# qurAI-amsterdam/SuperResolution_aniso_MRI

Hardware: AMD Instinct MI355X
Metric: training slices/sec (ae_combined, 160x160, latent=128) (higher is better)
Workload: dtype f32; 1 GPU; ACDC synthetic 12x(3x1x160x160) triplets, ae_combined latent=128 depth=32 scales=2, MSE synthesis loss (BASELINE configs[1]); global_batch_triplets=12, parallelism=dp1, init=reference Initializer, seed 892372, random weights, launch=captured HIP graph replay

## Files before the change

### superresolution_aniso_mri_amd/_hip.py

```python
import ctypes
import os
from ctypes import c_char_p, c_double, c_float, c_int, c_int64, c_size_t, c_void_p

import torch

_HERE = os.path.dirname(os.path.abspath(__file__))
LIB_PATH = os.path.join(_HERE, "libaesr_hip.so")
if os.environ.get("AESR_LIB"):
    import sys as _sys
    LIB_PATH = os.path.abspath(os.environ["AESR_LIB"])
    _sys.stderr.write("[aesr] AESR_LIB: loading the VARIANT library %s (not the shipped libaesr_hip.so)\n" % LIB_PATH)

P = c_void_p
IP = ctypes.POINTER(c_int)
FP = ctypes.POINTER(c_float)
DP = ctypes.POINTER(c_double)

class TripletDesc(ctypes.Structure):
    _fields_ = [("vol_off", ctypes.c_longlong), ("H", c_int), ("W", c_int), ("z_from", c_int), ("z_to", c_int), ("z_between", c_int),
                ("oy", c_int), ("ox", c_int), ("k", c_int), ("gain", c_float), ("cutoff", c_float)]


class WgradReduceJob(ctypes.Structure):
    _fields_ = [("workspace", c_void_p), ("dw", c_void_p), ("db", c_void_p), ("N", c_int), ("H", c_int), ("W", c_int), ("Cin", c_int),
# ... 124 lines not shown
    "aesr_comm_unique_id": (c_int, [c_char_p]),
    "aesr_comm_init": (c_int, [c_char_p, c_int, c_int, ctypes.POINTER(c_void_p)]),
    "aesr_comm_destroy": (c_int, [P]),
    "aesr_comm_abort": (c_int, [P]),
    "aesr_comm_allreduce": (c_int, [P, P, c_size_t, c_int, c_int, P]),
    "aesr_comm_allreduce_many": (c_int, [P, ctypes.POINTER(c_void_p), ctypes.POINTER(c_size_t), c_int, c_int, c_int, P]),
    "aesr_comm_broadcast": (c_int, [P, P, c_size_t, c_int, c_int, P]),
}
SIGNATURES_PREPROC = {
    "aesr_inplane_out_size": (c_int, [c_int, c_double]),
    "aesr_inplane_workspace_bytes": (c_size_t, [c_int, c_int]),
    "aesr_inplane_resample": (c_int, [P, P, P] + [c_int] * 5 + [DP, c_int, DP, c_int, IP, DP, IP, DP, c_int, P]),
}
SIGNATURES_DATAPREP = {
    "aesr_thick_slices_out_slices": (c_int, [c_int, c_int]),
    "aesr_thick_slices_store_bytes": (c_int, [c_int, P, P]),
    "aesr_thick_slices": (c_int, [P, P, c_int, c_int, c_int, c_int, DP, c_int, P]),
    "aesr_triplet_assemble_raw": (c_int, [P, ctypes.POINTER(TripletDesc), c_int, c_int, P, P, P]),
}
SIGNATURES_TRAIN = {
    "aesr_conv2d_cout1_bwd_workspace_floats": (c_size_t, [c_int]),
    "aesr_conv2d_cout1_bwd": (c_int, [P] * 8 + [c_int] * 5 + [c_float, c_int, c_float, P]),
}
SIGNATURES_BASELINES = {
    "aesr_z_expand_out_slices": (c_int, [c_int, c_int, c_int]),
    "aesr_z_expand_store_bytes": (c_int, [c_int, P, P]),
    "aesr_bspline_coef_bytes": (c_size_t, [c_int] * 4),
    "aesr_bspline_prefilter_z": (c_int, [P, P] + [c_int] * 4 + [P]),
    "aesr_z_expand": (c_int, [P, P, P] + [c_int] * 7 + [IP, DP, c_int, c_int, P]),
}
SIGNATURES_RESLICE = {
    "aesr_reslice_affine": (c_int, [P, P] + [c_int] * 7 + [DP, c_int, P]),
    "aesr_reslice_grid": (c_int, [P, P, P] + [c_int] * 7 + [c_int, P]),
}
SIGNATURES_SEG = {
    "aesr_softmax_dice_workspace_floats": (c_size_t, [c_int] * 4),
    "aesr_softmax_dice_fwd": (c_int, [P, P, c_size_t] + [P] * 5 + [c_int] * 4 + [P]),
    "aesr_softmax_dice_bwd": (c_int, [P, P, c_size_t, P, P, P] + [c_int] * 4 + [P]),
}
LLP = ctypes.POINTER(ctypes.c_longlong)
SIGNATURES_SURFACE = {
    "aesr_surface_workspace_bytes": (c_size_t, [c_int] * 5),
    "aesr_surface_borders": (c_int, [P, P, P, P] + [c_int] * 4 + [IP, c_int, c_int, c_int, P]),
    "aesr_surface_distances": (c_int, [P, P, LLP, P, c_size_t, P] + [c_int] * 6 + [DP, P]),
}
SURFACE_MAX_CLASSES, SURFACE_COUNTS, SURFACE_MAX_W = 8, 7, 4096
# ... 3 lines not shown
ZX_MAX_FACTOR, ZX_MAX_TAPS = 16, 10
P2P_HANDLE_BYTES, P2P_SLOTS = 64, 32
COMM_ID_BYTES = 128
COMM_F32, COMM_F64, COMM_SUM, COMM_MAX = 0, 1, 0, 1

ACT_NONE, ACT_LRELU, ACT_RELU, ACT_SIGMOID = 0, 1, 2, 3
BN_NONE, BN_POOL, BN_UP = 0, 1, 2
RS_POOL, RS_NEAREST, RS_BILINEAR = 1, 2, 3
BN_NWG = 512
REDUCE_MAX_JOBS = 16
MSE_NPART = 512
MSE3_WS = 3 * 256 + 1
LPIPS_NCH = 64


def _load():
    if not os.path.exists(LIB_PATH):
        raise RuntimeError(
            "libaesr_hip.so not found at %s -- build it with `python __graft_entry__.py` (or `make -C "
            "superresolution_aniso_mri_amd/csrc`). The HIP extension is mandatory: there is no CPU/eager fallback." % LIB_PATH)
    lib = ctypes.CDLL(LIB_PATH)
    for name, (res, args) in (list(SIGNATURES.items()) + list(SIGNATURES_PREPROC.items()) + list(SIGNATURES_DATAPREP.items())
                                   + list(SIGNATURES_TRAIN.items()) + list(SIGNATURES_BASELINES.items()) + list(SIGNATURES_RESLICE.items())
                                   + list(SIGNATURES_SEG.items()) + list(SIGNATURES_SURFACE.items())):
        fn = getattr(lib, name, None)
        if fn is None:
            raise RuntimeError("libaesr_hip.so does not export %s (stale build?)" % name)
        fn.restype, fn.argtypes = res, args
    return lib


lib = _load()


def last_error():
    return lib.aesr_last_error_string().decode("utf-8", "replace")


def check(rc, what):
    if rc != 0:
        raise RuntimeError("%s failed (code %d): %s" % (what, rc, last_error()))


def check_device_watchdogs(where):
    nb = int(lib.aesr_bn_fused1_timeouts())
    if nb:
        raise RuntimeError("%s: the one-launch BatchNorm kernel's grid barrier gave up %d time(s) in this process -- its workgroups were not all "
# ... 45 lines not shown
```

### superresolution_aniso_mri_amd/csrc/aesr_api.hip

```cpp
#include <stdarg.h>
#include <stdio.h>
#include <stdlib.h>
#include <string.h>

#include "../../include/aesr_hip.h"
#include "../../include/aesr_hip_dataprep.h"
#include "../../include/aesr_hip_train.h"
#include "aesr_kernels.h"
#include "conv_plan.h"

static thread_local char g_err[512] = "";
void aesr_set_error(const char* fmt, ...) {
    va_list ap;
    va_start(ap, fmt);
    vsnprintf(g_err, sizeof(g_err), fmt, ap);
    va_end(ap);
}

static bool fill_groups(BnGroups* gr, int G, const int* nstart_host) {
    if (G < 1 || G > 4 || !nstart_host) return false;
    gr->G = G;
    for (int i = 0; i <= G; ++i) gr->nstart[i] = nstart_host[i];
    for (int i = G + 1; i < 5; ++i) gr->nstart[i] = nstart_host[G];
    return true;
}

enum { GEOM_OK = 0, GEOM_FILTER, GEOM_DIMS, GEOM_SMALL };
static int conv_geom(int N, int H, int W, int Cin, int Cout, int KS, int pad, int* Ho, int* Wo) {
// ... 752 lines not shown
    AESR_CHECK_ARG(gout && y && mean && invstd && scale && sums && counts_host && coef && dgamma && dbeta && dpre &&
                       bn_bwd_args(&a, gout, y, mean, invstd, scale, coef, nullptr, dpre, N, H, W, C, mode, act, slope, G, nstart_host),
                   "aesr_bn_bwd_apply: bad arguments");
    if (aesr_bn_fused_ok(C, G))
        return aesr_launch_bn_bwd_finalize_apply(sums, counts_host, coef, dgamma, dbeta, G, a, (hipStream_t)stream);
    if (int e = aesr_launch_bn_bwd_finalize(sums, counts_host, coef, dgamma, dbeta, C, G, (hipStream_t)stream)) return e;
    return aesr_launch_bn_bwd_apply(a, (hipStream_t)stream);
}

int aesr_bn_bwd(const float* gout, const float* y, const float* mean, const float* invstd, const float* scale, float* partial,
                const double* counts_host, float* coef, float* dgamma, float* dbeta, float* dpre, int N, int H, int W, int C,
                int mode, int act, float slope, int G, const int* nstart_host, void* stream) {
    BnBwdArgs a;
    AESR_CHECK_ARG(gout && y && mean && invstd && scale && partial && counts_host && coef && dgamma && dbeta && dpre &&
                       bn_bwd_args(&a, gout, y, mean, invstd, scale, coef, partial, dpre, N, H, W, C, mode, act, slope, G, nstart_host),
                   "aesr_bn_bwd: bad arguments");
    AESR_CHECK_ARG((double)N * H * W < 2147483648.0, "aesr_bn_bwd: more than 2^31 pixels");
    if (int e = aesr_launch_bn_bwd_reduce(a, AESR_BN_NWG, (hipStream_t)stream)) return e;
    if (int e = aesr_launch_bn_bwd_reduce_finalize(partial, AESR_BN_NWG, counts_host, coef, dgamma, dbeta, C, G, (hipStream_t)stream))
        return e;
    return aesr_launch_bn_bwd_apply(a, (hipStream_t)stream);
}

int aesr_maxpool2_fwd(const float* x, float* out, int N, int H, int W, int C, void* stream) {
    AESR_CHECK_ARG(x && out && N > 0 && H >= 2 && W >= 2 && C % 4 == 0, "aesr_maxpool2_fwd: bad arguments (C %% 4 == 0, H,W >= 2)");
    return aesr_launch_maxpool2_fwd(x, out, N, H, W, C, (hipStream_t)stream);
}

int aesr_maxpool2_bwd(const float* gout, const float* x, const float* gadd, float* dx, int N, int H, int W, int C, int relu_mask,
                      void* stream) {
    AESR_CHECK_ARG(gout && x && dx && N > 0 && H >= 2 && W >= 2 && C % 4 == 0, "aesr_maxpool2_bwd: bad arguments");
    return aesr_launch_maxpool2_bwd(gout, x, gadd, dx, N, H, W, C, relu_mask, (hipStream_t)stream);
}

int aesr_scale_expand_fwd(const float* x, float* out4, size_t n, const float* ca_host, const float* cb_host, void* stream) {
    AESR_CHECK_ARG(x && out4 && ca_host && cb_host && n > 0 && n < ((size_t)1 << 29), "aesr_scale_expand_fwd: bad arguments");
    return aesr_launch_scale_expand(x, out4, (int)n, ca_host, cb_host, 0, (hipStream_t)stream);
}

int aesr_scale_expand_bwd(const float* d4, float* dx, size_t n, const float* ca_host, void* stream) {
    AESR_CHECK_ARG(d4 && dx && ca_host && n > 0 && n < ((size_t)1 << 29), "aesr_scale_expand_bwd: bad arguments");
    return aesr_launch_scale_expand(d4, dx, (int)n, ca_host, nullptr, 1, (hipStream_t)stream);
}

int aesr_lpips_tap_fwd(const float* f, const float* lin_w, float* partial, int B, int HW, int C, void* stream) {
    AESR_CHECK_ARG(f && lin_w && partial && B > 0 && HW > 0, "aesr_lpips_tap_fwd: bad arguments");
// ... 212 lines not shown
```

### superresolution_aniso_mri_amd/csrc/aesr_kernels.h

```cpp
#pragma once
#include "aesr_common.h"

struct IgemmArgs {
    const float* in; const float* wpk; const float* bias; const float* ysave; float* out;
    int N, H, W, Cin, CinP, Cout, CoutP, Ho, Wo, pad;
    int TI, TH, TW, tiles_y, tiles_x, nitems, dbg;
    int unused_;
    int ksplit;
    float* dbgbuf;
    int act, mask_act;
    float slope;
};
int aesr_launch_conv_igemm(const IgemmArgs& a, int KS, int NB, int MBW, hipStream_t st);
int aesr_launch_conv_ksplit_fixup(const float* partial, const float* bias, const float* ysave, float* out, size_t nelem, int Cout,
                                  int ksplit, int act, int mask_act, float slope, hipStream_t st);
int aesr_launch_pack_weights(const float* w, float* p, int Cout, int Cin, int KS, int KinP, int NoutP, int TN, int transpose, hipStream_t st);

struct WinoArgs {
    const float* in; const float* upk; const float* bias; const float* ysave; float* out;
    int N, H, W, Cin, CinP, Cout, CoutP;
    int TI, THt, TWt;
    int regs_y, regs_x, nitems;
    unsigned m_ncot, m_regs_x, m_regs_y;
    int act, mask_act;
// ... 163 lines not shown
bool aesr_bn_fused1_ok(int N, int H, int W, int C, int pool, int G, int backward);
unsigned aesr_bn_fused_timeouts_impl();
int aesr_launch_bn_stats(const float* y, float* partial, int HW, int C, const BnGroups& gr, int nwg, hipStream_t st);
int aesr_launch_bn_reduce(const float* partial, double* sums, int nwg, int C, int G, hipStream_t st);
int aesr_launch_bn_finalize(const double* sums, const double* counts, const float* gamma, const float* beta, float* rm, float* rv,
                            long long* nbt, float* mean, float* invstd, float* scale, float* shift, int C, int G, float momentum,
                            float eps, int train, int update_running, hipStream_t st);
int aesr_launch_bn_reduce_finalize(const float* partial, int nwg, const double* counts, const float* gamma, const float* beta,
                                   float* running_mean, float* running_var, long long* nbt, float* mean, float* invstd,
                                   float* scale, float* shift, int C, int G, float momentum, float eps, int update_running,
                                   hipStream_t st);
int aesr_launch_bn_bwd_reduce_finalize(const float* partial, int nwg, const double* counts, float* coef, float* dgamma,
                                       float* dbeta, int C, int G, hipStream_t st);
int aesr_launch_bn_apply(const BnApplyArgs& a, hipStream_t st);
int aesr_launch_bn_bwd_reduce(const BnBwdArgs& a, int nwg, hipStream_t st);
int aesr_launch_bn_bwd_finalize(const double* sums, const double* counts, float* coef, float* dgamma, float* dbeta, int C, int G, hipStream_t st);
int aesr_launch_bn_bwd_apply(const BnBwdArgs& a, hipStream_t st);
bool aesr_bn_fused_ok(int C, int G);
int aesr_launch_bn_finalize_apply(const double* sums, const double* counts, const float* gamma, const float* beta, float* running_mean,
                                  float* running_var, long long* nbt, float* mean, float* invstd, float* scale, float* shift, float momentum,
                                  float eps, int update_running, int G, const BnApplyArgs& a, hipStream_t st);
int aesr_launch_bn_bwd_finalize_apply(const double* sums, const double* counts, float* coef, float* dgamma, float* dbeta, int G,
                                      const BnBwdArgs& a, hipStream_t st);

int aesr_launch_lerp_fwd(const float* z, const float* af, const float* at, float* zmix, int B, size_t per, hipStream_t st);
int aesr_launch_lerp_bwd(const float* dmix, const float* af, const float* at, float* dz, int B, size_t per, hipStream_t st);
int aesr_launch_lerp_cat_fwd(const float* z, const float* af, const float* at, float* zcat, int B, size_t per, hipStream_t st);
int aesr_launch_interleave_clamp(const float* orig, const float* synth, float* out, int Z, int n, size_t per, float lo, float hi, hipStream_t st);
int aesr_launch_lerp_multi(const float* z, float* out, int Z, size_t per, const float* alphas, int n, float nslope, hipStream_t st);
int aesr_launch_lerp_cat_bwd(const float* g, const float* af, const float* at, float* dz, int B, size_t per, hipStream_t st);
int aesr_launch_mse_fwd(const float* a, const float* b, double* partial, int np, float* out, size_t n, hipStream_t st);
int aesr_launch_mse3_fwd(const float* const* a, const float* const* b, const size_t* n, const float* lam, double* ws, float* out, hipStream_t st);
int aesr_launch_mse3_bwd(const float* a1, const float* b1, size_t n1, const float* a2, const float* b2, size_t n2, const float* lam,
                         const float* g, float* d1, float* d2, hipStream_t st);
int aesr_launch_mse_bwd(const float* a, const float* b, const float* g, float* da, size_t n, hipStream_t st);
int aesr_launch_act_bwd(const float* dout, const float* y, float* dpre, size_t n, int act, float slope, hipStream_t st);
int aesr_launch_adam(float* p, float* g, float* m, float* v, float* state, size_t n, float lr, double beta1, double beta2,
                     float eps, float wd, int zero_g, hipStream_t st);


int aesr_launch_maxpool2_fwd(const float* x, float* out, int N, int H, int W, int C, hipStream_t st);
int aesr_launch_maxpool2_bwd(const float* gout, const float* x, const float* gadd, float* dx, int N, int H, int W, int C, int relu, hipStream_t st);
int aesr_launch_lpips_tap_fwd(const float* f, const float* lin, float* partial, int B, int HW, int C, hipStream_t st);
int aesr_launch_lpips_tap_bwd(const float* f, const float* lin, const float* gd, float* gf0, int B, int HW, int C, hipStream_t st);
int aesr_launch_lpips_finalize(const float* const* partials, const int* hw, int ntaps, float* d, int B, hipStream_t st);
int aesr_launch_scale_expand(const float* x, float* out4, int n, const float* ca, const float* cb, int backward, hipStream_t st);
// ... 24 lines not shown
```

### superresolution_aniso_mri_amd/csrc/bn.hip

```cpp
#include "bn_math.h"

enum { BN_MODE_NONE = 0, BN_MODE_POOL = 1, BN_MODE_UP = 2 };

__global__ __launch_bounds__(256) void bn_stats_kernel(const float* __restrict__ y, float* __restrict__ partial, int HW,
                                                       int C, BnGroups gr) {
    extern __shared__ __attribute__((aligned(16))) float red[];
    const int C4 = C >> 2, PL = 256 / C4;
    const int c4 = threadIdx.x % C4, pl = threadIdx.x / C4;
    const int g = blockIdx.y;
    const size_t p0 = (size_t)gr.nstart[g] * HW, p1 = (size_t)gr.nstart[g + 1] * HW;
    f32x4 s = {0.f, 0.f, 0.f, 0.f}, q = {0.f, 0.f, 0.f, 0.f};
    if (pl < PL) {
        for (size_t p = p0 + (size_t)blockIdx.x * PL + pl; p < p1; p += (size_t)gridDim.x * PL) {
            const f32x4 v = *(const f32x4*)(y + p * C + c4 * 4);
            s += v;
            q += v * v;
        }
        *(f32x4*)(red + (pl * 2 + 0) * C + c4 * 4) = s;
        *(f32x4*)(red + (pl * 2 + 1) * C + c4 * 4) = q;
    }
    __syncthreads();
    for (int o = threadIdx.x; o < 2 * C; o += 256) {
        float t = 0.f;
        for (int k = 0; k < PL; ++k) t += red[k * 2 * C + o];
// ... 273 lines not shown
        const f32x4 mu = *(const f32x4*)(a.mean + g * a.C + c4 * 4);
        const f32x4 iv = *(const f32x4*)(a.invstd + g * a.C + c4 * 4);
        const f32x4 sc = *(const f32x4*)(a.scale + g * a.C + c4 * 4);
        const f32x4 k1 = *(const f32x4*)(k_tab + (g * 2 + 0) * a.C + c4 * 4);
        const f32x4 k2 = *(const f32x4*)(k_tab + (g * 2 + 1) * a.C + c4 * 4);
        const f32x4 yv = *(const f32x4*)(a.y + idx * 4);
        const f32x4 gg = bn_gather_g_t<MODE>(a, n, yy, x, c4);
        *(f32x4*)(a.dpre + idx * 4) = bn_bwd_elem(yv, gg, mu, iv, sc, k1, k2, a.act, a.slope);
    }
}

template <int MODE>
__global__ __launch_bounds__(256) void bn_bwd_apply_kernel(BnBwdArgs a) { bn_bwd_apply_loop<MODE>(a, a.coef); }

template <int MODE>
__global__ __launch_bounds__(256) void bn_bwd_finalize_apply_kernel(const double* __restrict__ sums, BnCounts counts, float* __restrict__ coef,
                                                                    float* __restrict__ dgamma, float* __restrict__ dbeta, int G, BnBwdArgs a) {
    __shared__ __attribute__((aligned(16))) float s_k[2 * BN_FUSE_MAX];
    bn_bwd_tables<256>(sums, counts.c, G, a.C, blockIdx.x == 0, s_k, coef, dgamma, dbeta);
    __syncthreads();
    bn_bwd_apply_loop<MODE>(a, s_k);
}

static int bn_check_c(int C, const char* who) {
    if (C % 4 != 0 || 256 % (C / 4) != 0 || C > 1024) {
        aesr_set_error("%s: unsupported channel count %d (need C/4 | 256)", who, C);
        return AESR_ERR_ARG;
    }
    return AESR_OK;
}

static dim3 bn_stream_grid(size_t pixels, int C) {
    const size_t total = pixels * (C / 4);
    int grid = (int)((total + 255) / 256);
    if (grid > 4096) grid = 4096;
    return dim3(grid);
}

#define BN_LAUNCH_MODE(kernel, mode, grid, shm, st, ...)                                                       \
    do {                                                                                                       \
        if ((mode) == BN_MODE_POOL) hipLaunchKernelGGL(kernel<BN_MODE_POOL>, grid, dim3(256), shm, st, __VA_ARGS__); \
        else if ((mode) == BN_MODE_UP) hipLaunchKernelGGL(kernel<BN_MODE_UP>, grid, dim3(256), shm, st, __VA_ARGS__);  \
        else hipLaunchKernelGGL(kernel<0>, grid, dim3(256), shm, st, __VA_ARGS__);                             \
    } while (0)

int aesr_launch_bn_stats(const float* y, float* partial, int HW, int C, const BnGroups& gr, int nwg, hipStream_t st) {
// ... 92 lines not shown
}

bool aesr_bn_fused_ok(int C, int G) { return G * C <= BN_FUSE_MAX && G >= 1 && G <= 4; }

int aesr_launch_bn_finalize_apply(const double* sums, const double* counts, const float* gamma, const float* beta, float* running_mean,
                                  float* running_var, long long* nbt, float* mean, float* invstd, float* scale, float* shift, float momentum,
                                  float eps, int update_running, int G, const BnApplyArgs& a, hipStream_t st) {
    if (int e = bn_check_c(a.C, "bn_finalize_apply")) return e;
    const BnFinArgs f = bn_fin_args(counts, gamma, beta, running_mean, running_var, nbt, mean, invstd, scale, shift, a.C, G, momentum, eps, 1,
                                    update_running);
    hipLaunchKernelGGL(bn_finalize_apply_kernel, bn_stream_grid((size_t)a.N * a.Ho * a.Wo, a.C), dim3(256), 0, st, sums, f, a);
    AESR_LAUNCH_CHECK("bn_finalize_apply");
    return AESR_OK;
}

int aesr_launch_bn_bwd_finalize_apply(const double* sums, const double* counts, float* coef, float* dgamma, float* dbeta, int G,
                                      const BnBwdArgs& a, hipStream_t st) {
    if (int e = bn_check_c(a.C, "bn_bwd_finalize_apply")) return e;
    BN_LAUNCH_MODE(bn_bwd_finalize_apply_kernel, a.mode, bn_stream_grid((size_t)a.N * a.H * a.W, a.C), 0, st, sums, bn_counts(counts, G), coef,
                   dgamma, dbeta, G, a);
    AESR_LAUNCH_CHECK("bn_bwd_finalize_apply");
    return AESR_OK;
}
```

### superresolution_aniso_mri_amd/engine.py

```python
import os
from ctypes import c_float

import torch
import torch.nn as nn

from . import _hip
from ._hip import lib, ptr, stream, check

LRELU_SLOPE = 0.01


class KernelProfiler:

    def __init__(self):
        self.records = []

    def begin(self, kind, flops, nbytes=0.0):
        e0 = torch.cuda.Event(enable_timing=True)
        e1 = torch.cuda.Event(enable_timing=True)
        e0.record(torch.cuda.current_stream())
        self.records.append((kind, flops, nbytes, e0, e1))

    def end(self):
        self.records[-1][4].record(torch.cuda.current_stream())

    def summary(self):
        torch.cuda.synchronize()
        out = {}
        for kind, flops, nbytes, e0, e1 in self.records:
            d = out.setdefault(kind, {"launches": 0, "flops": 0.0, "bytes": 0.0, "ms": 0.0})
            d["launches"] += 1
            d["flops"] += flops
            d["bytes"] += nbytes
            d["ms"] += e0.elapsed_time(e1)
        return out


PROFILER = None
TRACE = None
FUSE_STEM = os.environ.get("AESR_FUSE_STEM", "1") != "0"
FUSE_COUT1_BWD = os.environ.get("AESR_FUSE_COUT1_BWD", "1") != "0"
USE_WINO = os.environ.get("AESR_WINO", "1") != "0"
FOLD_UPSAMPLE = os.environ.get("AESR_FOLD_UPSAMPLE", "1") != "0"
FUSE_EVAL_BN = os.environ.get("AESR_FUSE_EVAL_BN", "1") != "0"


def bn_fused_enabled():
    return os.environ.get("AESR_BN_FUSED", "1") != "0"


def bn_fused_pays(N, H, W, C):
    if N > int(os.environ.get("AESR_BN_FUSED_MAX_IMAGES", "9")):
        return False
    return float(N) * H * W * C * 4.0 <= float(os.environ.get("AESR_BN_FUSED_MAX_MB", "1000")) * 1e6


def wino_ok(cin, cout, ks, pad, transpose):
    return bool(USE_WINO and lib.aesr_conv2d_wino_supported(int(cin), int(cout), int(ks), int(pad), int(transpose)))


def wino_kind(n, h, w, cin, cout, transpose):
    k = lib.aesr_conv2d_wino_kernel(int(n), int(h), int(w), int(cin), int(cout), 3, 1, int(transpose))
    return {2: "conv_wino_res_f32", 3: "conv_wino_ring_f32"}.get(k, "conv_wino_f32")

# ... 350 lines not shown
                    check(lib.aesr_conv2d_smallcin_fwd(ptr(cur), ptr(s.mod.weight), ptr(bias), None, ptr(out), N, H, W,
                                                       s.cin, s.cout, s.ks, s.pad, act_k, _hip.ACT_NONE, s.slope, 0, 0,
                                                       None, None, stream()), "aesr_conv2d_smallcin_fwd")
                else:
                    raise NotImplementedError("conv with Cin=%d (neither <=4 nor a multiple of 4)" % s.cin)
                if save:
                    saved.append((cur, out, full_hw) if s.s2d else (cur, out))
                if TRACE is not None and not skip:
                    TRACE.append((self.seq, s.mod, act_k, out))
                cur, H, W, C = out, Ho, Wo, s.cout
            elif s.kind == "resample":
                if C % 4 != 0:
                    raise NotImplementedError("stand-alone pooling / upsampling of %d channels (needs a multiple of 4)" % C)
                Ho, Wo = s.out_hw(H, W)
                out = _empty((N, Ho, Wo, C), x)
                check(lib.aesr_resample2_fwd(ptr(cur), ptr(out), N, H, W, C, s.mode, stream()), "aesr_resample2_fwd")
                if save:
                    saved.append((cur,))
                cur, H, W = out, Ho, Wo
            else:
                bn = s.mod
                Ho, Wo = s.out_hw(H, W)
                out = _empty((N, Ho, Wo, C), x)
                _pb("bn_fwd", 0.0, 4.0 * (cur.numel() + out.numel()))
                st = self._bn_forward_stats(bn, cur, N, H, W, C, nstart, train, out, s.run_mode)
                if not st.pop("applied", False):
                    check(lib.aesr_bn_apply(ptr(cur), ptr(st["scale"]), ptr(st["shift"]), ptr(out), N, H, W, C, s.run_mode, G,
                                            _hip.int_array(nstart), stream()), "aesr_bn_apply")
                _pe()
                if save:
                    saved.append((cur, st))
                cur, H, W = out, Ho, Wo
        return cur, saved, steps

    def max_elems_per_image(self, H, W, C, first=0, last=None):
        return self.trace_shapes(H, W, C, first, last)[0]

    def trace_shapes(self, H, W, C, first=0, last=None):
        best = H * W * C
        for s in self.steps[first:last]:
            if s.kind == "conv":
                if s.s2d:
                    H, W = H // 2, W // 2
                elif s.in_up2:
                    H, W = 2 * H, 2 * W
                    H, W = s.out_hw(H, W)
                else:
                    H, W = s.out_hw(H, W)
# ... 8 lines not shown

    def _bn_barrier(self, dev):
        t = self.__dict__.get("_bn_bar")
        if t is None or t.device != torch.device(dev):
            if torch.cuda.is_current_stream_capturing():
                raise RuntimeError("one-launch BatchNorm: run the pass eagerly once before capturing it into a HIP graph")
            t = self._bn_bar = torch.zeros((int(lib.aesr_bn_fused1_barrier_words()),), device=dev, dtype=torch.int32)
        return t

    sync_p2p = None

    def _p2p_fits(self, N, H, W, C, run_mode, G, backward):
        p = self.sync_p2p
        if p is None or not bn_fused_enabled():
            return False
        nmax = max(N, int(round(N * p.nscale)))
        if float(nmax) * H * W * C * 4.0 > float(os.environ.get("AESR_P2P_MAX_MB", "12")) * 1e6:
            return False
        return bool(lib.aesr_bn_fused1_supported(nmax, H, W, C, run_mode, G, backward))

    sync_bn = None
    count_scale = 1.0

    def _bn_forward_stats(self, bn, y, N, H, W, C, nstart, train, out=None, run_mode=0):
        G = len(nstart) - 1
        dev = y.device
        st = {k: torch.empty((G, C), device=dev, dtype=torch.float32) for k in ("mean", "invstd", "scale", "shift")}
        use_batch = train or bn.running_mean is None
        momentum = 0.1 if bn.momentum is None else float(bn.momentum)
        update = bool(train and bn.track_running_stats and bn.running_mean is not None)
        if update:
            self._bn_updates = getattr(self, "_bn_updates", 0) + 1
        if not use_batch:
            ver = lambda t: (-1, 0) if t is None else (t._version, t.data_ptr())
            key = (self.weights_epoch, getattr(self, "_bn_updates", 0), ver(bn.weight), ver(bn.bias), ver(bn.running_mean), ver(bn.running_var),
                   G, str(dev))
            cache = self.__dict__.setdefault("_eval_bn", {})
            hit = cache.get(id(bn))
            if hit is not None and hit[0] == key and not torch.cuda.is_current_stream_capturing():
                return dict(hit[1])
        sums = None
        counts = [float((nstart[g + 1] - nstart[g]) * H * W) * self.count_scale for g in range(G)] if use_batch else None
        st["counts"] = counts
        if use_batch:
            partial = torch.empty((G * _hip.BN_NWG * 2 * C,), device=dev, dtype=torch.float32)
            local = (self.sync_bn is None and out is not None and bn_fused_enabled() and bn_fused_pays(N, H, W, C)
                     and lib.aesr_bn_fused1_supported(N, H, W, C, run_mode, G, 0))
            if local or (self.sync_bn is not None and out is not None and self._p2p_fits(N, H, W, C, run_mode, G, 0)):
                ws = torch.empty((lib.aesr_bn_fused1_workspace_floats(C, G),), device=dev, dtype=torch.float32)
                args = (ptr(y), ptr(out), ptr(ws), ptr(self._bn_barrier(dev)), _hip.double_array(counts), ptr(bn.weight), ptr(bn.bias),
                        ptr(bn.running_mean), ptr(bn.running_var), ptr(bn.num_batches_tracked), ptr(st["mean"]), ptr(st["invstd"]),
                        ptr(st["scale"]), ptr(st["shift"]), N, H, W, C, run_mode, G, _hip.int_array(nstart), momentum, float(bn.eps), int(update))
                if local:
                    check(lib.aesr_bn_fused1_fwd(*args, stream()), "aesr_bn_fused1_fwd")
                else:
                    p = self.sync_p2p
                    check(lib.aesr_bn_fused1_fwd_p2p(*args, p.peers, p.world, p.rank, p.next_slot(), ptr(p.gen), stream()), "aesr_bn_fused1_fwd_p2p")
                st["applied"] = True
                return st
            if self.sync_bn is None:
                check(lib.aesr_bn_stats_finalize(ptr(y), ptr(partial), _hip.double_array(counts), ptr(bn.weight), ptr(bn.bias),
                                                 ptr(bn.running_mean), ptr(bn.running_var), ptr(bn.num_batches_tracked),
                                                 ptr(st["mean"]), ptr(st["invstd"]), ptr(st["scale"]), ptr(st["shift"]), H * W, C,
                                                 G, _hip.int_array(nstart), momentum, float(bn.eps), int(update), stream()),
                      "aesr_bn_stats_finalize")
                return st
            sums = torch.empty((G, 2, C), device=dev, dtype=torch.float64)
            check(lib.aesr_bn_stats(ptr(y), ptr(partial), ptr(sums), H * W, C, G, _hip.int_array(nstart), stream()),
                  "aesr_bn_stats")
            self.sync_bn(sums)
            if out is not None and lib.aesr_bn_fused_supported(C, G):
                check(lib.aesr_bn_finalize_apply(ptr(sums), _hip.double_array(counts), ptr(bn.weight), ptr(bn.bias), ptr(bn.running_mean),
                                                 ptr(bn.running_var), ptr(bn.num_batches_tracked), ptr(st["mean"]), ptr(st["invstd"]),
                                                 ptr(st["scale"]), ptr(st["shift"]), ptr(y), ptr(out), N, H, W, C, run_mode, G,
                                                 _hip.int_array(nstart), momentum, float(bn.eps), int(update), stream()),
                      "aesr_bn_finalize_apply")
                st["applied"] = True
                return st
        check(lib.aesr_bn_finalize(ptr(sums), _hip.double_array(counts) if counts else None, ptr(bn.weight), ptr(bn.bias), ptr(bn.running_mean),
                                   ptr(bn.running_var), ptr(bn.num_batches_tracked), ptr(st["mean"]), ptr(st["invstd"]),
# ... 169 lines not shown
                    check(lib.aesr_depth_to_space2(ptr(dx), ptr(dfull), N, fh, fw, s.cin_full, stream()), "aesr_depth_to_space2")
                    dx = dfull
                g = dx
            elif s.kind == "resample":
                xin = saved[k][0]
                _, H, W, C = xin.shape
                prev = steps[k - 1]
                mask_act, mslope = (prev.act, prev.slope) if prev.kind in ("conv", "stemconv") else (_hip.ACT_NONE, 0.0)
                dx = _empty((ngrad, H, W, C), g)
                check(lib.aesr_resample2_bwd(ptr(g), ptr(xin) if mask_act != _hip.ACT_NONE else None, ptr(dx), ngrad, H, W, C,
                                             s.mode, mask_act, mslope, stream()), "aesr_resample2_bwd")
                g = dx
            else:
                y, st = saved[k]
                prev = steps[k - 1]
                _, H, W, C = y.shape
                N = ngrad
                dev = y.device
                partial = torch.empty((G * _hip.BN_NWG * 2 * C,), device=dev, dtype=torch.float32)
                nsa = _hip.int_array(ns)
                coef = torch.empty((G, 2, C), device=dev, dtype=torch.float32)
                dgamma, dbeta = self._grad_dst(s.mod.weight, grads), self._grad_dst(s.mod.bias, grads)
                dpre = _empty((N, H, W, C), y)
                _pb("bn_bwd", 0.0, 4.0 * (g.numel() + 2.0 * N * H * W * C))
                local = (self.sync_bn is None and bn_fused_enabled() and bn_fused_pays(N, H, W, C)
                         and lib.aesr_bn_fused1_supported(N, H, W, C, s.run_mode, G, 1))
                if local or (self.sync_bn is not None and self._p2p_fits(N, H, W, C, s.run_mode, G, 1)):
                    ws = torch.empty((lib.aesr_bn_fused1_workspace_floats(C, G),), device=dev, dtype=torch.float32)
                    args = (ptr(g), ptr(y), ptr(st["mean"]), ptr(st["invstd"]), ptr(st["scale"]), ptr(ws), ptr(self._bn_barrier(dev)),
                            _hip.double_array(st["counts"][:G]), ptr(coef), ptr(dgamma), ptr(dbeta), ptr(dpre), N, H, W, C, s.run_mode, prev.act,
                            prev.slope, G, nsa)
                    if local:
                        check(lib.aesr_bn_fused1_bwd(*args, stream()), "aesr_bn_fused1_bwd")
                    else:
                        p = self.sync_p2p
                        check(lib.aesr_bn_fused1_bwd_p2p(*args, p.peers, p.world, p.rank, p.next_slot(), ptr(p.gen), stream()), "aesr_bn_fused1_bwd_p2p")
                elif self.sync_bn is None:
                    check(lib.aesr_bn_bwd(ptr(g), ptr(y), ptr(st["mean"]), ptr(st["invstd"]), ptr(st["scale"]), ptr(partial),
                                          _hip.double_array(st["counts"][:G]), ptr(coef), ptr(dgamma), ptr(dbeta), ptr(dpre), N, H, W,
                                          C, s.run_mode, prev.act, prev.slope, G, nsa, stream()), "aesr_bn_bwd")
                else:
                    sums = torch.empty((G, 2, C), device=dev, dtype=torch.float64)
                    check(lib.aesr_bn_bwd_reduce(ptr(g), ptr(y), ptr(st["mean"]), ptr(st["invstd"]), ptr(partial), ptr(sums), N,
                                                 H, W, C, s.run_mode, G, nsa, stream()), "aesr_bn_bwd_reduce")
                    self.sync_bn(sums)
                    check(lib.aesr_bn_bwd_apply(ptr(g), ptr(y), ptr(st["mean"]), ptr(st["invstd"]), ptr(st["scale"]), ptr(sums),
                                                _hip.double_array(st["counts"][:G]), ptr(coef), ptr(dgamma), ptr(dbeta), ptr(dpre),
                                                N, H, W, C, s.run_mode, prev.act, prev.slope, G, nsa, stream()), "aesr_bn_bwd_apply")
                _pe()
                g = dpre
        return g


def prepare_weights(pairs):
    jobs, commits = [], []
    for runner, steps in pairs:
        j, c = runner._prep_jobs(steps)
        jobs += j
        commits += c
# ... 110 lines not shown
```

Measured before the change: 15740 slices/s.

## Materialize pooled tensor once in BN-pool forward and reuse it in backward reduce

For batch-norm steps that also 2x2-max-pool, the stats kernel now writes the pooled pre-normalisation tensor while it accumulates the statistics. A separate apply kernel then normalises only the smaller pooled tensor instead of re-reading the full-resolution input. The backward reduction reads the saved pooled tensor rather than recomputing the pool from the full activation. This costs an extra pooled-size buffer per BN-pool layer and adds new kernel paths, and it only applies when the single-launch fused BN path is not chosen and sync BN is off.

```diff
diff --git a/include/aesr_hip_bnpool.h b/include/aesr_hip_bnpool.h
--- /dev/null
+++ b/include/aesr_hip_bnpool.h
@@ -0,0 +1,31 @@
+#ifndef AESR_HIP_BNPOOL_H
+#define AESR_HIP_BNPOOL_H
+
+#include "aesr_hip.h"
+
+#ifdef __cplusplus
+extern "C" {
+#endif
+
+int aesr_bn_pool_supported(int N, int H, int W, int C, int G);
+
+int aesr_bn_pool_stats_finalize(const float* y,
+                                float* m,
+                                float* partial, const double* counts_host, const float* gamma, const float* beta,
+                                float* running_mean, float* running_var,
+                                int64_t* num_batches_tracked,
+                                float* mean, float* invstd, float* scale, float* shift,
+                                int N, int H, int W, int C, int G, const int* nstart_host, float momentum, float eps, int update_running,
+                                void* stream);
+
+int aesr_bn_pool_apply(const float* m, const float* scale, const float* shift, float* out , int N, int Ho, int Wo, int C,
+                       int G, const int* nstart_host, void* stream);
+
+int aesr_bn_pool_bwd(const float* gout, const float* y, const float* m, const float* mean, const float* invstd, const float* scale,
+                     float* partial, const double* counts_host, float* coef, float* dgamma, float* dbeta, float* dpre, int N, int H, int W,
+                     int C, int act, float slope, int G, const int* nstart_host, void* stream);
+
+#ifdef __cplusplus
+}
+#endif
+#endif
diff --git a/superresolution_aniso_mri_amd/_hip.py b/superresolution_aniso_mri_amd/_hip.py
--- a/superresolution_aniso_mri_amd/_hip.py
+++ b/superresolution_aniso_mri_amd/_hip.py
@@ -170,6 +170,12 @@
     "aesr_conv2d_cout1_bwd_workspace_floats": (c_size_t, [c_int]),
     "aesr_conv2d_cout1_bwd": (c_int, [P] * 8 + [c_int] * 5 + [c_float, c_int, c_float, P]),
 }
+SIGNATURES_BNPOOL = {
+    "aesr_bn_pool_supported": (c_int, [c_int] * 5),
+    "aesr_bn_pool_stats_finalize": (c_int, [P, P, P, DP] + [P] * 9 + [c_int] * 5 + [IP, c_float, c_float, c_int, P]),
+    "aesr_bn_pool_apply": (c_int, [P, P, P, P] + [c_int] * 5 + [IP, P]),
+    "aesr_bn_pool_bwd": (c_int, [P] * 7 + [DP] + [P] * 4 + [c_int] * 5 + [c_float, c_int, IP, P]),
+}
 SIGNATURES_BASELINES = {
     "aesr_z_expand_out_slices": (c_int, [c_int, c_int, c_int]),
     "aesr_z_expand_store_bytes": (c_int, [c_int, P, P]),
@@ -219,7 +225,7 @@
     lib = ctypes.CDLL(LIB_PATH)
     for name, (res, args) in (list(SIGNATURES.items()) + list(SIGNATURES_PREPROC.items()) + list(SIGNATURES_DATAPREP.items())
                                    + list(SIGNATURES_TRAIN.items()) + list(SIGNATURES_BASELINES.items()) + list(SIGNATURES_RESLICE.items())
-                                   + list(SIGNATURES_SEG.items()) + list(SIGNATURES_SURFACE.items())):
+                                   + list(SIGNATURES_SEG.items()) + list(SIGNATURES_SURFACE.items()) + list(SIGNATURES_BNPOOL.items())):
         fn = getattr(lib, name, None)
         if fn is None:
             raise RuntimeError("libaesr_hip.so does not export %s (stale build?)" % name)
diff --git a/superresolution_aniso_mri_amd/csrc/aesr_api.hip b/superresolution_aniso_mri_amd/csrc/aesr_api.hip
--- a/superresolution_aniso_mri_amd/csrc/aesr_api.hip
+++ b/superresolution_aniso_mri_amd/csrc/aesr_api.hip
@@ -4,6 +4,7 @@
 #include <string.h>
 
 #include "../../include/aesr_hip.h"
+#include "../../include/aesr_hip_bnpool.h"
 #include "../../include/aesr_hip_dataprep.h"
 #include "../../include/aesr_hip_train.h"
 #include "aesr_kernels.h"
@@ -802,6 +803,62 @@
     return aesr_launch_bn_bwd_apply(a, (hipStream_t)stream);
 }
 
+int aesr_bn_pool_supported(int N, int H, int W, int C, int G) {
+    if (C < 4 || C % 4 != 0 || C > 1024 || 256 % (C / 4) != 0) return 0;
+    if (H < 2 || W < 2 || G < 1 || G > 4 || N < G) return 0;
+    return (double)N * H * W < 2147483648.0 ? 1 : 0;
+}
+
+static bool bn_pool_groups(BnGroups* gr, int N, int H, int W, int C, int G, const int* nstart_host) {
+    if (!aesr_bn_pool_supported(N, H, W, C, G) || !fill_groups(gr, G, nstart_host)) return false;
+    if (gr->nstart[0] != 0 || gr->nstart[G] != N) return false;
+    for (int g = 0; g < G; ++g)
+        if (gr->nstart[g + 1] <= gr->nstart[g]) return false;
+    return true;
+}
+
+int aesr_bn_pool_stats_finalize(const float* y, float* m, float* partial, const double* counts_host, const float* gamma, const float* beta,
+                                float* running_mean, float* running_var, int64_t* num_batches_tracked, float* mean, float* invstd,
+                                float* scale, float* shift, int N, int H, int W, int C, int G, const int* nstart_host, float momentum,
+                                float eps, int update_running, void* stream) {
+    BnPoolStatsArgs a;
+    memset(&a, 0, sizeof(a));
+    AESR_CHECK_ARG(y && m && partial && counts_host && gamma && beta && mean && invstd && scale && shift,
+                   "aesr_bn_pool_stats_finalize: null pointer");
+    AESR_CHECK_ARG(bn_pool_groups(&a.gr, N, H, W, C, G, nstart_host),
+                   "aesr_bn_pool_stats_finalize: N=%d H=%d W=%d C=%d G=%d or the group table is not supported (aesr_bn_pool_supported)", N, H, W, C, G);
+    a.y = y; a.m = m; a.partial = partial; a.H = H; a.W = W; a.C = C; a.Ho = H / 2; a.Wo = W / 2;
+    if (int e = aesr_launch_bn_pool_stats(a, AESR_BN_NWG, (hipStream_t)stream)) return e;
+    return aesr_launch_bn_reduce_finalize(partial, AESR_BN_NWG, counts_host, gamma, beta, running_mean, running_var,
+                                          (long long*)num_batches_tracked, mean, invstd, scale, shift, C, G, momentum, eps,
+                                          update_running && running_mean && running_var, (hipStream_t)stream);
+}
+
+int aesr_bn_pool_apply(const float* m, const float* scale, const float* shift, float* out, int N, int Ho, int Wo, int C, int G,
+                       const int* nstart_host, void* stream) {
+    BnGroups gr;
+    AESR_CHECK_ARG(m && scale && shift && out, "aesr_bn_pool_apply: null pointer");
+    AESR_CHECK_ARG(Ho >= 1 && Wo >= 1 && (double)Ho * Wo < 536870912.0 && bn_pool_groups(&gr, N, 2 * Ho, 2 * Wo, C, G, nstart_host),
+                   "aesr_bn_pool_apply: N=%d Ho=%d Wo=%d C=%d G=%d or the group table is not supported (aesr_bn_pool_supported)", N, Ho, Wo, C, G);
+    return aesr_launch_bn_pool_apply(m, scale, shift, out, Ho * Wo, C, gr, (hipStream_t)stream);
+}
+
+int aesr_bn_pool_bwd(const float* gout, const float* y, const float* m, const float* mean, const float* invstd, const float* scale,
+                     float* partial, const double* counts_host, float* coef, float* dgamma, float* dbeta, float* dpre, int N, int H, int W,
+                     int C, int act, float slope, int G, const int* nstart_host, void* stream) {
+    BnBwdArgs a;
+    AESR_CHECK_ARG(gout && y && m && mean && invstd && scale && partial && counts_host && coef && dgamma && dbeta && dpre,
+                   "aesr_bn_pool_bwd: null pointer");
+    AESR_CHECK_ARG(act >= ACT_NONE && act <= ACT_SIGMOID, "aesr_bn_pool_bwd: unknown activation code %d", act);
+    AESR_CHECK_ARG(bn_bwd_args(&a, gout, y, mean, invstd, scale, coef, partial, dpre, N, H, W, C, AESR_BN_POOL, act, slope, G, nstart_host) &&
+                       bn_pool_groups(&a.gr, N, H, W, C, G, nstart_host),
+                   "aesr_bn_pool_bwd: N=%d H=%d W=%d C=%d G=%d or the group table is not supported (aesr_bn_pool_supported)", N, H, W, C, G);
+    if (int e = aesr_launch_bn_pool_bwd_reduce(gout, m, mean, invstd, partial, a.Ho * a.Wo, C, a.gr, AESR_BN_NWG, (hipStream_t)stream)) return e;
+    if (int e = aesr_launch_bn_bwd_reduce_finalize(partial, AESR_BN_NWG, counts_host, coef, dgamma, dbeta, C, G, (hipStream_t)stream))
+        return e;
+    return aesr_launch_bn_bwd_apply(a, (hipStream_t)stream);
+}
+
 int aesr_maxpool2_fwd(const float* x, float* out, int N, int H, int W, int C, void* stream) {
     AESR_CHECK_ARG(x && out && N > 0 && H >= 2 && W >= 2 && C % 4 == 0, "aesr_maxpool2_fwd: bad arguments (C %% 4 == 0, H,W >= 2)");
     return aesr_launch_maxpool2_fwd(x, out, N, H, W, C, (hipStream_t)stream);
diff --git a/superresolution_aniso_mri_amd/csrc/aesr_kernels.h b/superresolution_aniso_mri_amd/csrc/aesr_kernels.h
--- a/superresolution_aniso_mri_amd/csrc/aesr_kernels.h
+++ b/superresolution_aniso_mri_amd/csrc/aesr_kernels.h
@@ -209,6 +209,18 @@
                                   float eps, int update_running, int G, const BnApplyArgs& a, hipStream_t st);
 int aesr_launch_bn_bwd_finalize_apply(const double* sums, const double* counts, float* coef, float* dgamma, float* dbeta, int G,
                                       const BnBwdArgs& a, hipStream_t st);
+struct BnPoolStatsArgs {
+    const float* y; float* m; float* partial;
+    int H, W, C, Ho, Wo;
+    BnGroups gr;
+    unsigned long long m_win, m_wo;
+    int k_win, k_wo;
+};
+int aesr_launch_bn_pool_stats(const BnPoolStatsArgs& a, int nwg, hipStream_t st);
+int aesr_launch_bn_pool_apply(const float* m, const float* scale, const float* shift, float* out, int HoWo, int C, const BnGroups& gr,
+                              hipStream_t st);
+int aesr_launch_bn_pool_bwd_reduce(const float* gout, const float* m, const float* mean, const float* invstd, float* partial, int HoWo, int C,
+                                   const BnGroups& gr, int nwg, hipStream_t st);
 
 int aesr_launch_lerp_fwd(const float* z, const float* af, const float* at, float* zmix, int B, size_t per, hipStream_t st);
 int aesr_launch_lerp_bwd(const float* dmix, const float* af, const float* at, float* dz, int B, size_t per, hipStream_t st);
diff --git a/superresolution_aniso_mri_amd/csrc/bn.hip b/superresolution_aniso_mri_amd/csrc/bn.hip
--- a/superresolution_aniso_mri_amd/csrc/bn.hip
+++ b/superresolution_aniso_mri_amd/csrc/bn.hip
@@ -319,6 +319,135 @@
     bn_bwd_apply_loop<MODE>(a, s_k);
 }
 
+
+template <bool ODD>
+__global__ __launch_bounds__(256) void bn_stats_kernel_pool(BnPoolStatsArgs a) {
+    extern __shared__ __attribute__((aligned(16))) float red[];
+    const int C = a.C, C4 = C >> 2, PL = 256 / C4;
+    const int c4 = threadIdx.x % C4, pl = threadIdx.x / C4;
+    const int g = blockIdx.y;
+    const unsigned HoWo = a.Ho * a.Wo;
+    f32x4 s = {0.f, 0.f, 0.f, 0.f}, q = {0.f, 0.f, 0.f, 0.f};
+    if (pl < PL) {
+        const unsigned S = gridDim.x * PL;
+        const size_t row = (size_t)a.W * C;
+        const unsigned w1 = a.gr.nstart[g + 1] * HoWo;
+        for (unsigned w = a.gr.nstart[g] * HoWo + blockIdx.x * PL + pl; w < w1; w += S) {
+            const unsigned n = bn_fastdiv(w, a.m_win, a.k_win);
+            const unsigned rem = w - n * HoWo;
+            const unsigned py = bn_fastdiv(rem, a.m_wo, a.k_wo), px = rem - py * a.Wo;
+            const float* b = a.y + (((size_t)n * a.H + 2 * py) * a.W + 2 * px) * C + c4 * 4;
+            const f32x4 v00 = *(const f32x4*)b, v01 = *(const f32x4*)(b + C);
+            const f32x4 v10 = *(const f32x4*)(b + row), v11 = *(const f32x4*)(b + row + C);
+            s += (v00 + v01) + (v10 + v11);
+            q += (v00 * v00 + v01 * v01) + (v10 * v10 + v11 * v11);
+            *(f32x4*)(a.m + (size_t)w * C + c4 * 4) = bn_pool2x2(v00, v01, v10, v11);
+        }
+        const unsigned Tc = (a.W & 1) ? a.H : 0, T = Tc + ((a.H & 1) ? 2 * a.Wo : 0);
+        if (ODD && T) {
+            const unsigned t1 = a.gr.nstart[g + 1] * T;
+            for (unsigned t = a.gr.nstart[g] * T + blockIdx.x * PL + pl; t < t1; t += S) {
+                const unsigned n = t / T, r = t - n * T;
+                const unsigned yy = r < Tc ? r : a.H - 1, x = r < Tc ? a.W - 1 : r - Tc;
+                const f32x4 v = *(const f32x4*)(a.y + (((size_t)n * a.H + yy) * a.W + x) * C + c4 * 4);
+                s += v;
+                q += v * v;
+            }
+        }
+        *(f32x4*)(red + (pl * 2 + 0) * C + c4 * 4) = s;
+        *(f32x4*)(red + (pl * 2 + 1) * C + c4 * 4) = q;
+    }
+    __syncthreads();
+    for (int o = threadIdx.x; o < 2 * C; o += 256) {
+        float t = 0.f;
+        for (int k = 0; k < PL; ++k) t += red[k * 2 * C + o];
+        a.partial[((size_t)g * gridDim.x + blockIdx.x) * 2 * C + o] = t;
+    }
+}
+
+template <int U>
+__global__ __launch_bounds__(256) void bn_apply_kernel_pooled(const float* __restrict__ m, const float* __restrict__ scale,
+                                                              const float* __restrict__ shift, float* __restrict__ out, size_t per, int C,
+                                                              BnGroups gr) {
+    const int c4 = threadIdx.x % (C >> 2);
+    const size_t total = gr.nstart[gr.G] * per, b1 = gr.nstart[1] * per, b2 = gr.nstart[2] * per, b3 = gr.nstart[3] * per;
+    const size_t S = (size_t)gridDim.x * 256;
+    size_t idx = (size_t)blockIdx.x * 256 + threadIdx.x;
+    for (; idx + (U - 1) * S < total; idx += U * S) {
+        f32x4 v[U], sc[U], sh[U];
+#pragma unroll
+        for (int u = 0; u < U; ++u) {
+            const size_t i = idx + u * S;
+            const int g = (int)(i >= b1) + (int)(i >= b2) + (int)(i >= b3);
+            v[u] = *(const f32x4*)(m + i * 4);
+            sc[u] = *(const f32x4*)(scale + g * C + c4 * 4);
+            sh[u] = *(const f32x4*)(shift + g * C + c4 * 4);
+        }
+#pragma unroll
+        for (int u = 0; u < U; ++u) *(f32x4*)(out + (idx + u * S) * 4) = bn_fwd_elem(v[u], sc[u], sh[u]);
+    }
+    for (; idx < total; idx += S) {
+        const int g = (int)(idx >= b1) + (int)(idx >= b2) + (int)(idx >= b3);
+        const f32x4 sc = *(const f32x4*)(scale + g * C + c4 * 4);
+        const f32x4 sh = *(const f32x4*)(shift + g * C + c4 * 4);
+        *(f32x4*)(out + idx * 4) = bn_fwd_elem(*(const f32x4*)(m + idx * 4), sc, sh);
+    }
+}
+
+template <int U>
+__global__ __launch_bounds__(256) void bn_bwd_reduce_kernel_pooled(const float* __restrict__ gout, const float* __restrict__ m,
+                                                                   const float* __restrict__ mean, const float* __restrict__ invstd,
+                                                                   float* __restrict__ partial, unsigned HoWo, int C, BnGroups gr) {
+    extern __shared__ __attribute__((aligned(16))) float red[];
+    const int C4 = C >> 2, PL = 256 / C4;
+    const int c4 = threadIdx.x % C4, pl = threadIdx.x / C4;
+    const int g = blockIdx.y;
+    const unsigned w1 = gr.nstart[g + 1] * HoWo;
+    const f32x4 mu = *(const f32x4*)(mean + g * C + c4 * 4);
+    const f32x4 iv = *(const f32x4*)(invstd + g * C + c4 * 4);
+    f32x4 s1 = {0.f, 0.f, 0.f, 0.f}, s2 = {0.f, 0.f, 0.f, 0.f};
+    if (pl < PL) {
+        const unsigned S = gridDim.x * PL;
+        unsigned w = gr.nstart[g] * HoWo + blockIdx.x * PL + pl;
+        f32x4 a1[U], a2[U];
+#pragma unroll
+        for (int u = 0; u < U; ++u) a1[u] = a2[u] = (f32x4){0.f, 0.f, 0.f, 0.f};
+        for (; w + (U - 1) * S < w1; w += U * S) {
+            f32x4 mv[U], gq[U];
+#pragma unroll
+            for (int u = 0; u < U; ++u) {
+                const size_t o = (size_t)(w + u * S) * C + c4 * 4;
+                gq[u] = *(const f32x4*)(gout + o);
+                mv[u] = *(const f32x4*)(m + o);
+            }
+#pragma unroll
+            for (int u = 0; u < U; ++u) {
+                a1[u] += gq[u];
+                a2[u] += gq[u] * ((mv[u] - mu) * iv);
+            }
+        }
+        for (; w < w1; w += S) {
+            const size_t o = (size_t)w * C + c4 * 4;
+            const f32x4 gg = *(const f32x4*)(gout + o);
+            s1 += gg;
+            s2 += gg * ((*(const f32x4*)(m + o) - mu) * iv);
+        }
+#pragma unroll
+        for (int u = 0; u < U; ++u) {
+            s1 += a1[u];
+            s2 += a2[u];
+        }
+        *(f32x4*)(red + (pl * 2 + 0) * C + c4 * 4) = s1;
+        *(f32x4*)(red + (pl * 2 + 1) * C + c4 * 4) = s2;
+    }
+    __syncthreads();
+    for (int o = threadIdx.x; o < 2 * C; o += 256) {
+        float t = 0.f;
+        for (int k = 0; k < PL; ++k) t += red[k * 2 * C + o];
+        partial[((size_t)g * gridDim.x + blockIdx.x) * 2 * C + o] = t;
+    }
+}
+
 static int bn_check_c(int C, const char* who) {
     if (C % 4 != 0 || 256 % (C / 4) != 0 || C > 1024) {
         aesr_set_error("%s: unsupported channel count %d (need C/4 | 256)", who, C);
@@ -457,3 +586,35 @@
     AESR_LAUNCH_CHECK("bn_bwd_finalize_apply");
     return AESR_OK;
 }
+
+int aesr_launch_bn_pool_stats(const BnPoolStatsArgs& a_in, int nwg, hipStream_t st) {
+    BnPoolStatsArgs a = a_in;
+    if (int e = bn_check_c(a.C, "bn_pool_stats")) return e;
+    bn_magic((unsigned)(a.Ho * a.Wo), &a.m_win, &a.k_win);
+    bn_magic((unsigned)a.Wo, &a.m_wo, &a.k_wo);
+    const int PL = 256 / (a.C / 4);
+    const size_t shm = (size_t)PL * 2 * a.C * sizeof(float);
+    if ((a.H | a.W) & 1) hipLaunchKernelGGL(bn_stats_kernel_pool<true>, dim3(nwg, a.gr.G), dim3(256), shm, st, a);
+    else hipLaunchKernelGGL(bn_stats_kernel_pool<false>, dim3(nwg, a.gr.G), dim3(256), shm, st, a);
+    AESR_LAUNCH_CHECK("bn_pool_stats");
+    return AESR_OK;
+}
+
+int aesr_launch_bn_pool_apply(const float* m, const float* scale, const float* shift, float* out, int HoWo, int C, const BnGroups& gr,
+                              hipStream_t st) {
+    if (int e = bn_check_c(C, "bn_pool_apply")) return e;
+    hipLaunchKernelGGL(bn_apply_kernel_pooled<2>, bn_stream_grid((size_t)gr.nstart[gr.G] * HoWo, C), dim3(256), 0, st, m, scale, shift, out,
+                       (size_t)HoWo * (C / 4), C, gr);
+    AESR_LAUNCH_CHECK("bn_pool_apply");
+    return AESR_OK;
+}
+
+int aesr_launch_bn_pool_bwd_reduce(const float* gout, const float* m, const float* mean, const float* invstd, float* partial, int HoWo, int C,
+                                   const BnGroups& gr, int nwg, hipStream_t st) {
+    if (int e = bn_check_c(C, "bn_pool_bwd_reduce")) return e;
+    const int PL = 256 / (C / 4);
+    hipLaunchKernelGGL(bn_bwd_reduce_kernel_pooled<4>, dim3(nwg, gr.G), dim3(256), (size_t)PL * 2 * C * sizeof(float), st, gout, m, mean, invstd,
+                       partial, (unsigned)HoWo, C, gr);
+    AESR_LAUNCH_CHECK("bn_pool_bwd_reduce");
+    return AESR_OK;
+}
diff --git a/superresolution_aniso_mri_amd/engine.py b/superresolution_aniso_mri_amd/engine.py
--- a/superresolution_aniso_mri_amd/engine.py
+++ b/superresolution_aniso_mri_amd/engine.py
@@ -40,6 +40,7 @@
 TRACE = None
 FUSE_STEM = os.environ.get("AESR_FUSE_STEM", "1") != "0"
 FUSE_COUT1_BWD = os.environ.get("AESR_FUSE_COUT1_BWD", "1") != "0"
+BN_POOL_ONCE = os.environ.get("AESR_BN_POOL_ONCE", "1") != "0"
 USE_WINO = os.environ.get("AESR_WINO", "1") != "0"
 FOLD_UPSAMPLE = os.environ.get("AESR_FOLD_UPSAMPLE", "1") != "0"
 FUSE_EVAL_BN = os.environ.get("AESR_FUSE_EVAL_BN", "1") != "0"
@@ -436,8 +437,9 @@
                 bn = s.mod
                 Ho, Wo = s.out_hw(H, W)
                 out = _empty((N, Ho, Wo, C), x)
-                _pb("bn_fwd", 0.0, 4.0 * (cur.numel() + out.numel()))
-                st = self._bn_forward_stats(bn, cur, N, H, W, C, nstart, train, out, s.run_mode)
+                m = _empty((N, Ho, Wo, C), x) if self._bn_pool_once(bn, N, H, W, C, s.run_mode, G, train) else None
+                _pb("bn_fwd", 0.0, 4.0 * (cur.numel() + out.numel() + (0 if m is None else m.numel())))
+                st = self._bn_forward_stats(bn, cur, N, H, W, C, nstart, train, out, s.run_mode, m)
                 if not st.pop("applied", False):
                     check(lib.aesr_bn_apply(ptr(cur), ptr(st["scale"]), ptr(st["shift"]), ptr(out), N, H, W, C, s.run_mode, G,
                                             _hip.int_array(nstart), stream()), "aesr_bn_apply")
@@ -492,7 +494,16 @@
     sync_bn = None
     count_scale = 1.0
 
-    def _bn_forward_stats(self, bn, y, N, H, W, C, nstart, train, out=None, run_mode=0):
+    def _bn_one_launch(self, N, H, W, C, run_mode, G, backward):
+        return bool(self.sync_bn is None and bn_fused_enabled() and bn_fused_pays(N, H, W, C)
+                    and lib.aesr_bn_fused1_supported(N, H, W, C, run_mode, G, backward))
+
+    def _bn_pool_once(self, bn, N, H, W, C, run_mode, G, train):
+        if not BN_POOL_ONCE or run_mode != _hip.BN_POOL or self.sync_bn is not None or not (train or bn.running_mean is None):
+            return False
+        return not self._bn_one_launch(N, H, W, C, run_mode, G, 0) and bool(lib.aesr_bn_pool_supported(N, H, W, C, G))
+
+    def _bn_forward_stats(self, bn, y, N, H, W, C, nstart, train, out=None, run_mode=0, m=None):
         G = len(nstart) - 1
         dev = y.device
         st = {k: torch.empty((G, C), device=dev, dtype=torch.float32) for k in ("mean", "invstd", "scale", "shift")}
@@ -514,8 +525,7 @@
         st["counts"] = counts
         if use_batch:
             partial = torch.empty((G * _hip.BN_NWG * 2 * C,), device=dev, dtype=torch.float32)
-            local = (self.sync_bn is None and out is not None and bn_fused_enabled() and bn_fused_pays(N, H, W, C)
-                     and lib.aesr_bn_fused1_supported(N, H, W, C, run_mode, G, 0))
+            local = out is not None and self._bn_one_launch(N, H, W, C, run_mode, G, 0)
             if local or (self.sync_bn is not None and out is not None and self._p2p_fits(N, H, W, C, run_mode, G, 0)):
                 ws = torch.empty((lib.aesr_bn_fused1_workspace_floats(C, G),), device=dev, dtype=torch.float32)
                 args = (ptr(y), ptr(out), ptr(ws), ptr(self._bn_barrier(dev)), _hip.double_array(counts), ptr(bn.weight), ptr(bn.bias),
@@ -526,6 +536,18 @@
                 else:
                     p = self.sync_p2p
                     check(lib.aesr_bn_fused1_fwd_p2p(*args, p.peers, p.world, p.rank, p.next_slot(), ptr(p.gen), stream()), "aesr_bn_fused1_fwd_p2p")
+                st["applied"] = True
+                return st
+            if m is not None:
+                nsa = _hip.int_array(nstart)
+                check(lib.aesr_bn_pool_stats_finalize(ptr(y), ptr(m), ptr(partial), _hip.double_array(counts), ptr(bn.weight), ptr(bn.bias),
+                                                      ptr(bn.running_mean), ptr(bn.running_var), ptr(bn.num_batches_tracked),
+                                                      ptr(st["mean"]), ptr(st["invstd"]), ptr(st["scale"]), ptr(st["shift"]), N, H, W, C,
+                                                      G, nsa, momentum, float(bn.eps), int(update), stream()),
+                      "aesr_bn_pool_stats_finalize")
+                check(lib.aesr_bn_pool_apply(ptr(m), ptr(st["scale"]), ptr(st["shift"]), ptr(out), N, H // 2, W // 2, C, G, nsa, stream()),
+                      "aesr_bn_pool_apply")
+                st["m"] = m
                 st["applied"] = True
                 return st
             if self.sync_bn is None:
@@ -741,9 +763,9 @@
                 coef = torch.empty((G, 2, C), device=dev, dtype=torch.float32)
                 dgamma, dbeta = self._grad_dst(s.mod.weight, grads), self._grad_dst(s.mod.bias, grads)
                 dpre = _empty((N, H, W, C), y)
-                _pb("bn_bwd", 0.0, 4.0 * (g.numel() + 2.0 * N * H * W * C))
-                local = (self.sync_bn is None and bn_fused_enabled() and bn_fused_pays(N, H, W, C)
-                         and lib.aesr_bn_fused1_supported(N, H, W, C, s.run_mode, G, 1))
+                local = self._bn_one_launch(N, H, W, C, s.run_mode, G, 1)
+                m = st.get("m") if (self.sync_bn is None and not local and lib.aesr_bn_pool_supported(N, H, W, C, G)) else None
+                _pb("bn_bwd", 0.0, 4.0 * (g.numel() + 2.0 * N * H * W * C + (0 if m is None else g.numel())))
                 if local or (self.sync_bn is not None and self._p2p_fits(N, H, W, C, s.run_mode, G, 1)):
                     ws = torch.empty((lib.aesr_bn_fused1_workspace_floats(C, G),), device=dev, dtype=torch.float32)
                     args = (ptr(g), ptr(y), ptr(st["mean"]), ptr(st["invstd"]), ptr(st["scale"]), ptr(ws), ptr(self._bn_barrier(dev)),
@@ -754,6 +776,10 @@
                     else:
                         p = self.sync_p2p
                         check(lib.aesr_bn_fused1_bwd_p2p(*args, p.peers, p.world, p.rank, p.next_slot(), ptr(p.gen), stream()), "aesr_bn_fused1_bwd_p2p")
+                elif m is not None:
+                    check(lib.aesr_bn_pool_bwd(ptr(g), ptr(y), ptr(m), ptr(st["mean"]), ptr(st["invstd"]), ptr(st["scale"]), ptr(partial),
+                                               _hip.double_array(st["counts"][:G]), ptr(coef), ptr(dgamma), ptr(dbeta), ptr(dpre), N, H, W,
+                                               C, prev.act, prev.slope, G, nsa, stream()), "aesr_bn_pool_bwd")
                 elif self.sync_bn is None:
                     check(lib.aesr_bn_bwd(ptr(g), ptr(y), ptr(st["mean"]), ptr(st["invstd"]), ptr(st["scale"]), ptr(partial),
                                           _hip.double_array(st["counts"][:G]), ptr(coef), ptr(dgamma), ptr(dbeta), ptr(dpre), N, H, W,
```

Result: faster. 16050 slices/s (median of 6 runs) (+2.0%).
